# nv-tlabs/GEN3C

Measured on AMD Instinct MI355X. Metric: denoise-steps/sec (121x1280x704 latent, Cosmos-7B), higher is better.
Workload: dtype bf16

## Files before the change

### gen3c_amd/build.py

```python
from __future__ import annotations

import os
import shutil
import subprocess
import sys
from concurrent.futures import ThreadPoolExecutor
from pathlib import Path

ROOT = Path(__file__).resolve().parent
CSRC = ROOT / "csrc"
LIBDIR = ROOT / "lib"
OBJDIR = LIBDIR / "obj"
LIB = LIBDIR / "libgen3c_hip.so"
ARCH = "gfx950"
PER_FILE_FLAGS = {"attention.hip": ("-fno-slp-vectorize",)}


def _hipcc() -> str:
    for cand in (os.environ.get("HIPCC"), shutil.which("hipcc"), "/opt/rocm/bin/hipcc"):
        if cand and Path(cand).exists():
            return cand
    raise RuntimeError("hipcc not found (ROCm toolchain is required to build the gen3c_amd HIP library)")


# ... 5 lines not shown


AUDITED = ("attention", "gemm", "attention_d512")


def _asm_audit(hipcc: str, flags: list, objdir: Path, verbose: bool) -> None:
    root = ROOT.parent
    if not (root / "tools" / "asm_audit.py").exists():
        print("gen3c_amd.build: tools/asm_audit.py not found - inline-asm register audit skipped", file=sys.stderr)
        return
    if str(root) not in sys.path:
        sys.path.insert(0, str(root))
    from tools import asm_audit

    def to_asm(stem: str) -> str:
        out = objdir / (stem + ".audit.s")
        cmd = [hipcc, *flags, *PER_FILE_FLAGS.get(stem + ".hip", ()), "-S", "--cuda-device-only", str(CSRC / (stem + ".hip")), "-o", str(out)]
        if verbose:
            print(" ".join(cmd), flush=True)
        r = subprocess.run(cmd, capture_output=True, text=True)
        if r.returncode != 0:
            raise RuntimeError(f"hipcc -S failed for {stem}.hip:\n{r.stderr}")
        text = out.read_text()
        out.unlink()
        return text

    with ThreadPoolExecutor(max_workers=len(AUDITED)) as ex:
        attn, gemm, d512 = ex.map(to_asm, AUDITED)
    import contextlib
    import io
    buf = io.StringIO()
    with contextlib.redirect_stdout(buf):
        findings = asm_audit.audit(attn) + asm_audit.audit_gemm_w4(gemm) + asm_audit.audit_gemm_w4e(gemm) + asm_audit.audit_attn_d512(d512)
    if verbose:
        print(buf.getvalue())
    if findings:
        raise RuntimeError("inline-asm register audit failed (tools/asm_audit.py):\n" + "\n".join(findings))


def build(verbose: bool = False, force: bool = False, extra_flags: tuple = (), suffix: str = "", audit: bool = True) -> Path:
    hipcc = _hipcc()
    objdir = LIBDIR / ("obj" + suffix)
    lib = LIBDIR / f"libgen3c_hip{suffix}.so"
    objdir.mkdir(parents=True, exist_ok=True)
    headers = sorted(CSRC.glob("*.hpp")) + sorted((ROOT.parent / "include").glob("*.h"))
    sources = sorted(CSRC.glob("*.hip"))
    flags = [f"--offload-arch={ARCH}", "-O3", "-std=c++17", "-fPIC", "-ffp-contract=off", f"-I{ROOT.parent / 'include'}", "-Wall",
             "-Wno-unused-function", *extra_flags]

    stamp = objdir / "asm_audit.ok"
    stale = [src.stem for src in sources if force or _newer(src, objdir / (src.stem + ".o"), headers)]
    audit_future = None
    audit_pool = None
    if audit and not suffix and (not stamp.exists() or any(s_ in AUDITED for s_ in stale)):
        stamp.unlink(missing_ok=True)
        audit_pool = ThreadPoolExecutor(max_workers=1)
        audit_future = audit_pool.submit(_asm_audit, hipcc, flags, objdir, verbose)

    def compile_one(src: Path) -> Path:
        obj = objdir / (src.stem + ".o")
        if src.stem in stale:
            cmd = [hipcc, *flags, *PER_FILE_FLAGS.get(src.name, ()), "-c", str(src), "-o", str(obj)]
            if verbose:
                print(" ".join(cmd), flush=True)
            r = subprocess.run(cmd, capture_output=True, text=True)
            if r.returncode != 0:
# ... 26 lines not shown
```

### gen3c_amd/csrc/attention.hip

```cpp
#include "common.hpp"
#include <stdlib.h>
#include <mutex>
#include <type_traits>

namespace {

constexpr int HD = 128;
constexpr int QB = 32;
constexpr int NWAVES = 8;
constexpr int BQ = QB * NWAVES;
constexpr int KVB = 64;
constexpr int NTHREADS = 64 * NWAVES;

struct AttnParams {
    const bf16_t* Q; int64_t q_row, q_batch, q_head;
    const bf16_t* K; int64_t k_row, k_batch, k_head;
    const bf16_t* Vt; int64_t vt_row, vt_batch, vt_head;
    bf16_t* O; int64_t o_row, o_batch, o_head;
    int Sq, Skv;
    float scale_log2;
    int vt_seg_len;
    int64_t vt_seg_stride;
    int grid_q, n_hb, n_heads, xcd_heads;
    float* O32;
// ... 380 lines not shown
    const float l_tot = xor32_sum(l_run);
    const float inv = 1.0f / l_tot;
    if (q_ok) {
        bf16_t* orow = Ob + (int64_t)q_idx * p.o_row;
#pragma unroll
        for (int d = 0; d < 4; ++d)
#pragma unroll
            for (int q4 = 0; q4 < 4; ++q4) {
                bf16x4 o;
#pragma unroll
                for (int e = 0; e < 4; ++e) o[e] = f32_to_bf16(accO[d][4 * q4 + e] * inv);
                *reinterpret_cast<bf16x4*>(orow + 32 * d + 8 * q4 + 4 * g) = o;
            }
    }
}


template <int OFF> G3_DEVICE void lds_read_frag(bf16x8& dst, uint32_t addr) {
    static_assert(OFF >= 0 && OFF < 65536, "ds_read offset field is 16 bits");
    asm volatile("ds_read_b128 %0, %1 offset:%2" : "=v"(dst) : "v"(addr), "n"(OFF));
}
G3_DEVICE uint32_t lds_addr_flip128(uint32_t a) {
    uint32_t r;
    asm volatile("v_xor_b32 %0, 0x80, %1" : "=v"(r) : "v"(a));
    return r;
}
template <int N> G3_DEVICE void lds_wait_frag(bf16x8& frag) { asm volatile("s_waitcnt lgkmcnt(%1)" : "+v"(frag) : "n"(N)); }

#define G3_SGB(mask, n) __builtin_amdgcn_sched_group_barrier((mask), (n), 0)
constexpr int SGB_VALU = 0x2, SGB_MFMA = 0x8, SGB_DSR = 0x100, SGB_TRANS = 0x400;

#ifndef G3_AB_ATTN_ABLATE
#define G3_AB_ATTN_ABLATE 0
#endif
template <int CTX, int QA, int QBV, bool FOLD, bool MW = false, int MW_RD = 4, int MW_KREGS = 8>
__global__ __launch_bounds__(NTHREADS, 2) void flash_attn_fwd_v3_kernel(AttnParams p) {
    constexpr bool CP = (CTX & 2) != 0;
    extern __shared__ __attribute__((aligned(16))) char smem_raw[];
    bf16_t* sK = reinterpret_cast<bf16_t*>(smem_raw);
    bf16_t* sV = sK + 2 * KVB * HD;

    const int tid = threadIdx.x;
    const int lane = tid & 63;
    const int wave = tid >> 6;
    const int l31 = lane & 31;
    const int g = lane >> 5;
    const int Skv = p.kv_dense > 0 ? p.kv_dense : p.Skv;
    const int head = blockIdx.y;
    const int batch = blockIdx.z;

    const bf16_t* Qb = p.Q + batch * p.q_batch + head * p.q_head;
    const bf16_t* Kb = p.K + batch * p.k_batch + head * p.k_head;
    const bf16_t* Vb = p.Vt + batch * p.vt_batch + head * p.vt_head;
    bf16_t* Ob = p.O + batch * p.o_batch + head * p.o_head;

    const int q_idx = blockIdx.x * BQ + wave * QB + l31;
    const bool q_ok = q_idx < p.Sq;
    bf16x8 qf[8];
    {
        const bf16_t* qrow = Qb + (int64_t)(q_ok ? q_idx : 0) * p.q_row + 8 * g;
#pragma unroll
        for (int ks = 0; ks < 8; ++ks) qf[ks] = q_ok ? load_bf16x8(qrow + 16 * ks) : zero_bf16x8();
        if (p.q_norm_w) {
            float ss = 0.f;
#pragma unroll
            for (int ks = 0; ks < 8; ++ks)
// ... 735 lines not shown
```

### gen3c_amd/csrc/attention_w4.hpp

```cpp

constexpr int W4_WAVES = 4;
constexpr int W4_THREADS = 64 * W4_WAVES;
constexpr int W4_BQ = 64 * W4_WAVES;
constexpr int W4_QBASE = 128;

#define W4_OWNED_AGPRS "a0","a1","a2","a3","a4","a5","a6","a7","a8","a9","a10","a11","a12","a13","a14","a15","a16","a17","a18","a19","a20","a21","a22","a23","a24","a25","a26","a27","a28","a29","a30","a31","a32","a33","a34","a35","a36","a37","a38","a39","a40","a41","a42","a43","a44","a45","a46","a47","a48","a49","a50","a51","a52","a53","a54","a55","a56","a57","a58","a59","a60","a61","a62","a63","a64","a65","a66","a67","a68","a69","a70","a71","a72","a73","a74","a75","a76","a77","a78","a79","a80","a81","a82","a83","a84","a85","a86","a87","a88","a89","a90","a91","a92","a93","a94","a95","a96","a97","a98","a99","a100","a101","a102","a103","a104","a105","a106","a107","a108","a109","a110","a111","a112","a113","a114","a115","a116","a117","a118","a119","a120","a121","a122","a123","a124","a125","a126","a127","a128","a129","a130","a131","a132","a133","a134","a135","a136","a137","a138","a139","a140","a141","a142","a143","a144","a145","a146","a147","a148","a149","a150","a151","a152","a153","a154","a155","a156","a157","a158","a159","a160","a161","a162","a163","a164","a165","a166","a167","a168","a169","a170","a171","a172","a173","a174","a175","a176","a177","a178","a179","a180","a181","a182","a183","a184","a185","a186","a187","a188","a189","a190","a191"

template <int R> G3_DEVICE void w4_acc_zero() { asm volatile("v_accvgpr_write_b32 a%c0, 0" ::"n"(R) : W4_OWNED_AGPRS); }
template <int R> G3_DEVICE void w4_acc_write(uint32_t v) { asm volatile("v_accvgpr_write_b32 a%c1, %0" ::"v"(v), "n"(R) : W4_OWNED_AGPRS); }
template <int R> G3_DEVICE float w4_acc_read() {
    float v;
    asm volatile("v_accvgpr_read_b32 %0, a%c1" : "=v"(v) : "n"(R) : W4_OWNED_AGPRS);
    return v;
}
template <int R> G3_DEVICE void w4_acc_scale(float alpha) {
    float t;
    asm volatile("v_accvgpr_read_b32 %0, a%c2\n\tv_mul_f32 %0, %0, %1\n\tv_accvgpr_write_b32 a%c2, %0" : "=&v"(t) : "v"(alpha), "n"(R) : W4_OWNED_AGPRS);
}
G3_DEVICE void w4_fence_acc() { asm volatile("s_nop 7\n\ts_nop 3" ::: W4_OWNED_AGPRS); }
G3_DEVICE void w4_fence_v(f32x16& a, f32x16& b, f32x16& c, f32x16& d) { asm volatile("s_nop 7\n\ts_nop 3" : "+v"(a), "+v"(b), "+v"(c), "+v"(d)); }

template <int QI, int WAIT> G3_DEVICE void w4_qk(f32x16& S, const bf16x8& kfrag) {
    if constexpr (WAIT >= 0)
        asm volatile("s_waitcnt lgkmcnt(%c4)\n\tv_mfma_f32_32x32x16_bf16 %0, %1, a[%c2:%c3], %0"
                     : "+v"(S) : "v"(kfrag), "n"(W4_QBASE + 4 * QI), "n"(W4_QBASE + 4 * QI + 3), "n"(WAIT) : W4_OWNED_AGPRS);
    else
        asm volatile("v_mfma_f32_32x32x16_bf16 %0, %1, a[%c2:%c3], %0" : "+v"(S) : "v"(kfrag), "n"(W4_QBASE + 4 * QI), "n"(W4_QBASE + 4 * QI + 3) : W4_OWNED_AGPRS);
}
template <int QI, int WAIT> G3_DEVICE void w4_qk0(f32x16& S, const bf16x8& kfrag, const f32x16& c) {
    if constexpr (WAIT >= 0)
        asm volatile("s_waitcnt lgkmcnt(%c5)\n\tv_mfma_f32_32x32x16_bf16 %0, %1, a[%c3:%c4], %2"
                     : "=&v"(S) : "v"(kfrag), "v"(c), "n"(W4_QBASE + 4 * QI), "n"(W4_QBASE + 4 * QI + 3), "n"(WAIT) : W4_OWNED_AGPRS);
    else
        asm volatile("v_mfma_f32_32x32x16_bf16 %0, %1, a[%c3:%c4], %2" : "=&v"(S) : "v"(kfrag), "v"(c), "n"(W4_QBASE + 4 * QI), "n"(W4_QBASE + 4 * QI + 3) : W4_OWNED_AGPRS);
}
template <int OB, int WAIT> G3_DEVICE void w4_pv(const bf16x8& vfrag, const u32x4& pfrag) {
    if constexpr (WAIT >= 0)
        asm volatile("s_waitcnt lgkmcnt(%c4)\n\tv_mfma_f32_32x32x16_bf16 a[%c2:%c3], %0, %1, a[%c2:%c3]" ::"v"(vfrag), "v"(pfrag), "n"(16 * OB), "n"(16 * OB + 15), "n"(WAIT) : W4_OWNED_AGPRS);
    else
        asm volatile("v_mfma_f32_32x32x16_bf16 a[%c2:%c3], %0, %1, a[%c2:%c3]" ::"v"(vfrag), "v"(pfrag), "n"(16 * OB), "n"(16 * OB + 15) : W4_OWNED_AGPRS);
}
G3_DEVICE void w4_dma_piece(uint32_t lds_dst, const char* sbase, uint32_t voff) {
    if (G3_AB_ATTN_ABLATE & 128) return;
    asm volatile("s_mov_b32 m0, %0\n\ts_nop 0\n\tglobal_load_lds_dwordx4 %1, %2" ::"s"(lds_dst), "v"(voff), "s"(sbase) : "memory");
}
template <int OFF> G3_DEVICE void lds_read_frag_flip128(bf16x8& dst, uint32_t addr) {
    uint32_t tmp;
    asm volatile("v_xor_b32 %1, 0x80, %2\n\tds_read_b128 %0, %1 offset:%3" : "=v"(dst), "=&v"(tmp) : "v"(addr), "n"(OFF));
}

#if G3_AB_ATTN_ABLATE & 16
#define W4_UNIT(k) "v_mov_b32 %[k" #k "], 0\n\t"
#else
#define W4_UNIT(k)                                                                                                                      \
    "v_exp_f32 %[a" #k "], %[x" #k "]\n\tv_exp_f32 %[b" #k "], %[y" #k "]\n\tv_add_f32 %[p" #k "], %[p" #k "], %[a" #k "]\n\t"      \
    "v_add_f32 %[r" #k "], %[r" #k "], %[b" #k "]\n\tv_cvt_pk_bf16_f32 %[k" #k "], %[a" #k "], %[b" #k "]\n\t"
#endif
#if G3_AB_ATTN_ABLATE & 32
#define W4_READ ""
#else
#define W4_READ "ds_read_b128 %[nf], %[addr] offset:%c[off]\n\t"
#endif
#ifdef G3_AB_ATTN_EXTRA_NOP
#define W4_WAIT "s_nop 0\n\ts_waitcnt lgkmcnt(%c[wn])\n\t"
#else
#define W4_WAIT "s_waitcnt lgkmcnt(%c[wn])\n\t"
#endif
#define W4_QK(h) "v_mfma_f32_32x32x16_bf16 %[s" #h "], %[f], a[%c[q" #h "]:%c[e" #h "]], %[s" #h "]\n\t"
#define W4_QK0(h) "v_mfma_f32_32x32x16_bf16 %[s" #h "], %[f], a[%c[q" #h "]:%c[e" #h "]], %[c" #h "]\n\t"
#define W4_PV(h) "v_mfma_f32_32x32x16_bf16 a[%c[o" #h "]:%c[g" #h "]], %[f], %[pf" #h "], a[%c[o" #h "]:%c[g" #h "]]\n\t"

struct W4Unit {
    float x, y;
};

template <int QI0, int OFF, int WN, bool INIT, bool TWO>
G3_DEVICE void w4_step_qk(bf16x8& nf, uint32_t addr, const bf16x8& f, f32x16& s0, f32x16& s1, const f32x16& c0, const f32x16& c1, float x1, float y1,
                          uint32_t& k1, float& p1, float& r1, float x2, float y2, uint32_t& k2, float& p2, float& r2) {
    float a1, b1, a2, b2;
    constexpr int q0 = W4_QBASE + 4 * QI0, q1 = W4_QBASE + 4 * (8 + QI0);
#define W4_A_OUT_COMMON [nf] "=&v"(nf), [a1] "=&v"(a1), [b1] "=&v"(b1), [k1] "=&v"(k1), [p1] "+v"(p1), [r1] "+v"(r1)
#define W4_A_OUT_TWO , [a2] "=&v"(a2), [b2] "=&v"(b2), [k2] "=&v"(k2), [p2] "+v"(p2), [r2] "+v"(r2)
#define W4_A_IN_COMMON [f] "v"(f), [addr] "v"(addr), [x1] "v"(x1), [y1] "v"(y1), [off] "n"(OFF), [wn] "n"(WN), [q0] "n"(q0), [e0] "n"(q0 + 3), [q1] "n"(q1), [e1] "n"(q1 + 3)
    if constexpr (INIT && TWO)
        asm volatile(W4_READ W4_WAIT W4_QK0(0) W4_UNIT(1) W4_QK0(1) W4_UNIT(2)
                     : W4_A_OUT_COMMON W4_A_OUT_TWO, [s0] "=&v"(s0), [s1] "=&v"(s1)
                     : W4_A_IN_COMMON, [x2] "v"(x2), [y2] "v"(y2), [c0] "v"(c0), [c1] "v"(c1) : W4_OWNED_AGPRS);
    else if constexpr (INIT && !TWO)
        asm volatile(W4_READ W4_WAIT W4_QK0(0) W4_UNIT(1) W4_QK0(1)
// ... 351 lines not shown
```

### gen3c_amd/csrc/attention_w4b.hpp

```cpp

#ifndef G3_ATTENTION_W4B_HELPERS
#define G3_ATTENTION_W4B_HELPERS
#define W4B_RING_AGPRS "a192","a193","a194","a195","a196","a197","a198","a199","a200","a201","a202","a203","a204","a205","a206","a207","a208","a209","a210","a211","a212","a213","a214","a215","a216","a217","a218","a219","a220","a221","a222","a223","a224","a225","a226","a227","a228","a229","a230","a231","a232","a233","a234","a235","a236","a237","a238","a239","a240","a241","a242","a243","a244","a245","a246","a247","a248","a249","a250","a251","a252","a253","a254","a255"
#define W4B_OWNED W4_OWNED_AGPRS, W4B_RING_AGPRS
constexpr int W4B_RING0 = 192;
constexpr int W4B_D = 6;

#if G3_AB_ATTN_ABLATE & 32
#define W4B_READ ""
#else
#define W4B_READ "ds_read_b128 a[%c[ra]:%c[rb]], %[addr] offset:%c[off]\n\t"
#endif
#define W4B_QK(h) "v_mfma_f32_32x32x16_bf16 %[s" #h "], a[%c[fa]:%c[fb]], a[%c[q" #h "]:%c[e" #h "]], %[s" #h "]\n\t"
#define W4B_QK0(h) "v_mfma_f32_32x32x16_bf16 %[s" #h "], a[%c[fa]:%c[fb]], a[%c[q" #h "]:%c[e" #h "]], %[c" #h "]\n\t"
#define W4B_PV(h) "v_mfma_f32_32x32x16_bf16 a[%c[o" #h "]:%c[g" #h "]], a[%c[fa]:%c[fb]], %[pf" #h "], a[%c[o" #h "]:%c[g" #h "]]\n\t"
#if G3_AB_ATTN_ABLATE & 128
#define W4B_M0 ""
#define W4B_DMA ""
#else
#define W4B_M0 "s_mov_b32 m0, %[m0v]\n\t"
#define W4B_DMA "global_load_lds_dwordx4 %[voff], %[sbase]\n\t"
#endif
#if G3_AB_ATTN_ABLATE & 256
#define W4B_MAXP(k) ""
// ... 21 lines not shown
    constexpr int q0 = W4_QBASE + 4 * ks, q1 = W4_QBASE + 4 * (8 + ks);
    constexpr int fa = W4B_RING0 + 4 * (I & 15), ra = W4B_RING0 + 4 * ((I + W4B_D) & 15);
#define W4B_A_OUT [a1] "+v"(a1), [b1] "+v"(b1), [k1] "=&v"(k1), [p1] "+v"(p1), [r1] "+v"(r1)
#define W4B_A_IN [addr] "v"(addr), [x1] "v"(x1), [y1] "v"(y1), [off] "n"(ROFF), [wn] "n"(WN), [q0] "n"(q0), [e0] "n"(q0 + 3), [q1] "n"(q1), [e1] "n"(q1 + 3), \
                 [fa] "n"(fa), [fb] "n"(fa + 3), [ra] "n"(ra), [rb] "n"(ra + 3)
    static_assert(READ, "region A always reads ahead");
    if constexpr (INIT && DMA)
        asm volatile(W4B_M0 W4B_READ W4_WAIT W4B_QK0(0) W4_UNIT(1) W4B_DMA W4B_QK0(1)
                     : W4B_A_OUT, [s0] "=&v"(s0), [s1] "=&v"(s1) : W4B_A_IN, [c0] "v"(c0), [c1] "v"(c1), [m0v] "s"(m0v), [voff] "v"(voff), [sbase] "s"(sbase)
                     : "memory");
    else if constexpr (!INIT && DMA)
        asm volatile(W4B_M0 W4B_READ W4_WAIT W4B_QK(0) W4_UNIT(1) W4B_DMA W4B_QK(1)
                     : W4B_A_OUT, [s0] "+v"(s0), [s1] "+v"(s1) : W4B_A_IN, [m0v] "s"(m0v), [voff] "v"(voff), [sbase] "s"(sbase) : "memory");
    else if constexpr (INIT && !DMA && EXTRA == 1)
        asm volatile(W4B_READ W4_WAIT W4B_QK0(0) W4_UNIT(1) W4B_QK0(1) W4B_XA
                     : W4B_A_OUT, [s0] "=&v"(s0), [s1] "=&v"(s1), [a2] "=&v"(*a2), [b2] "=&v"(*b2), [pe] "+v"(*pe)
                     : W4B_A_IN, [c0] "v"(c0), [c1] "v"(c1), [x2] "v"(x2), [y2] "v"(y2));
    else if constexpr (INIT && !DMA)
        asm volatile(W4B_READ W4_WAIT W4B_QK0(0) W4_UNIT(1) W4B_QK0(1)
                     : W4B_A_OUT, [s0] "=&v"(s0), [s1] "=&v"(s1) : W4B_A_IN, [c0] "v"(c0), [c1] "v"(c1));
    else if constexpr (EXTRA == 1)
        asm volatile(W4B_READ W4_WAIT W4B_QK(0) W4_UNIT(1) W4B_QK(1) W4B_XA
                     : W4B_A_OUT, [s0] "+v"(s0), [s1] "+v"(s1), [a2] "=&v"(*a2), [b2] "=&v"(*b2), [pe] "+v"(*pe) : W4B_A_IN, [x2] "v"(x2), [y2] "v"(y2));
    else if constexpr (EXTRA == 2)
        asm volatile(W4B_READ W4_WAIT W4B_QK(0) W4_UNIT(1) W4B_QK(1) W4B_XB
                     : W4B_A_OUT, [s0] "+v"(s0), [s1] "+v"(s1), [k2] "=&v"(*k2), [pe] "+v"(*pe) : W4B_A_IN, [a2] "v"(*a2), [b2] "v"(*b2));
    else
        asm volatile(W4B_READ W4_WAIT W4B_QK(0) W4_UNIT(1) W4B_QK(1) : W4B_A_OUT, [s0] "+v"(s0), [s1] "+v"(s1) : W4B_A_IN);
    static_assert(EXTRA == 0 || (!DMA && !(INIT && EXTRA == 2)), "w4b_step_qk: extra half units only on steps without an LDS-DMA piece");
#undef W4B_A_OUT
#undef W4B_A_IN
}

template <int I, int ROFF, bool READ, int WN, bool UNIT, int MX>
G3_DEVICE void w4b_step_pv(uint32_t addr, const u32x4& pf0, const u32x4& pf1, float x1, float y1, uint32_t& k1, float& p1, float& r1, float& mx, float& my,
                           float ma0, float mb0, float mc0, float md0, float ma1, float mb1, float mc1, float md1, float ma2, float mb2, float mc2, float md2,
                           float& a1, float& b1) {
    constexpr int D = I & 3;
    constexpr int o0 = 16 * D, o1 = 16 * (4 + D);
    constexpr int fa = W4B_RING0 + 4 * ((16 + I) & 15), ra = W4B_RING0 + 4 * ((16 + I + W4B_D) & 15);
#define W4B_B_IN [pf0] "v"(pf0), [pf1] "v"(pf1), [wn] "n"(WN), [o0] "n"(o0), [g0] "n"(o0 + 15), [o1] "n"(o1), [g1] "n"(o1 + 15), [fa] "n"(fa), [fb] "n"(fa + 3)
#define W4B_B_RD [addr] "v"(addr), [off] "n"(ROFF), [ra] "n"(ra), [rb] "n"(ra + 3)
#define W4B_B_UO [a1] "+v"(a1), [b1] "+v"(b1), [k1] "=&v"(k1), [p1] "+v"(p1), [r1] "+v"(r1)
#define W4B_B_UI [x1] "v"(x1), [y1] "v"(y1)
#define W4B_B_M0 [ma0] "v"(ma0), [mb0] "v"(mb0), [mc0] "v"(mc0), [md0] "v"(md0)
    if constexpr (READ && UNIT && MX == 0)
        asm volatile(W4B_READ W4_WAIT W4B_PV(0) W4_UNIT(1) W4B_PV(1) : W4B_B_UO : W4B_B_IN, W4B_B_RD, W4B_B_UI);
    else if constexpr (READ && UNIT && MX == 1)
        asm volatile(W4B_READ W4_WAIT W4B_PV(0) W4_UNIT(1) W4B_PV(1) W4B_MAXP0(0) : W4B_B_UO, [mx] "=&v"(mx), [my] "=&v"(my) : W4B_B_IN, W4B_B_RD, W4B_B_UI, W4B_B_M0);
    else if constexpr (READ && UNIT && MX == 2)
        asm volatile(W4B_READ W4_WAIT W4B_PV(0) W4_UNIT(1) W4B_PV(1) W4B_MAXP(0) : W4B_B_UO, [mx] "+v"(mx), [my] "+v"(my) : W4B_B_IN, W4B_B_RD, W4B_B_UI, W4B_B_M0);
    else if constexpr (!READ && UNIT && MX == 1)
        asm volatile(W4_WAIT W4B_PV(0) W4_UNIT(1) W4B_PV(1) W4B_MAXP0(0) : W4B_B_UO, [mx] "=&v"(mx), [my] "=&v"(my) : W4B_B_IN, W4B_B_UI, W4B_B_M0);
    else if constexpr (!READ && UNIT && MX == 2)
        asm volatile(W4_WAIT W4B_PV(0) W4_UNIT(1) W4B_PV(1) W4B_MAXP(0) : W4B_B_UO, [mx] "+v"(mx), [my] "+v"(my) : W4B_B_IN, W4B_B_UI, W4B_B_M0);
    else if constexpr (!READ && UNIT && MX == 0)
        asm volatile(W4_WAIT W4B_PV(0) W4_UNIT(1) W4B_PV(1) : W4B_B_UO : W4B_B_IN, W4B_B_UI);
    else if constexpr (!READ && !UNIT && MX == 3)
        asm volatile(W4_WAIT W4B_PV(0) W4B_MAXP(0) W4B_PV(1) W4B_MAXP(1) W4B_MAXP(2)
                     : [mx] "+v"(mx), [my] "+v"(my)
                     : W4B_B_IN, W4B_B_M0, [ma1] "v"(ma1), [mb1] "v"(mb1), [mc1] "v"(mc1), [md1] "v"(md1), [ma2] "v"(ma2), [mb2] "v"(mb2), [mc2] "v"(mc2), [md2] "v"(md2));
    else if constexpr (READ && !UNIT && MX == 3)
        asm volatile(W4B_READ W4_WAIT W4B_PV(0) W4B_MAXP(0) W4B_PV(1) W4B_MAXP(1) W4B_MAXP(2)
                     : [mx] "+v"(mx), [my] "+v"(my)
                     : W4B_B_IN, W4B_B_RD, W4B_B_M0, [ma1] "v"(ma1), [mb1] "v"(mb1), [mc1] "v"(mc1), [md1] "v"(md1), [ma2] "v"(ma2), [mb2] "v"(mb2), [mc2] "v"(mc2), [md2] "v"(md2));
    else if constexpr (READ && !UNIT && MX == 0)
        asm volatile(W4B_READ W4_WAIT W4B_PV(0) W4B_PV(1) : : W4B_B_IN, W4B_B_RD);
    else {
        static_assert(!READ && !UNIT && MX == 0, "w4b_step_pv: combination not laid out");
        asm volatile(W4_WAIT W4B_PV(0) W4B_PV(1) : : W4B_B_IN);
    }
#undef W4B_B_RD
#undef W4B_B_UO
#undef W4B_B_UI
#undef W4B_B_M0
}
template <int I, int WN, bool READ = false, int ROFF = 0>
G3_DEVICE void w4b_step_pv_fold(const u32x4& pf0, const u32x4& pf1, float& a0, float& b0, float& c0, float& d0, float& a1, float& b1, float& c1, float& d1, float& t0,
                                 float& t1, uint32_t addr = 0u) {
    constexpr int D = I & 3;
    constexpr int o0 = 16 * D, o1 = 16 * (4 + D);
    constexpr int fa = W4B_RING0 + 4 * ((16 + I) & 15), ra = W4B_RING0 + 4 * ((16 + I + W4B_D) & 15);
    if constexpr (READ && I == 14)
        asm volatile(W4B_READ W4_WAIT W4B_PV(0) "v_max3_f32 %[a0], %[a0], %[b0], %[c0]\n\tv_max3_f32 %[a1], %[a1], %[b1], %[c1]\n\tv_max_f32 %[a0], %[a0], %[d0]\n\tv_max_f32 %[a1], %[a1], %[d1]\n\t"
                     W4B_PV(1) "v_mov_b32 %[t0], %[a0]\n\tv_mov_b32 %[t1], %[a1]\n\t"
                     : [a0] "+v"(a0), [a1] "+v"(a1), [t0] "=&v"(t0), [t1] "=&v"(t1)
                     : W4B_B_IN, [b0] "v"(b0), [c0] "v"(c0), [d0] "v"(d0), [b1] "v"(b1), [c1] "v"(c1), [d1] "v"(d1), [addr] "v"(addr), [off] "n"(ROFF), [ra] "n"(ra), [rb] "n"(ra + 3));
    else if constexpr (READ)
        asm volatile(W4B_READ W4_WAIT W4B_PV(0) "v_permlane32_swap_b32 %[t0], %[a0]\n\tv_permlane32_swap_b32 %[t1], %[a1]\n\t" W4B_PV(1)
                     "v_max_f32 %[a0], %[a0], %[t0]\n\tv_max_f32 %[a1], %[a1], %[t1]\n\t"
                     : [a0] "+v"(a0), [a1] "+v"(a1), [t0] "+v"(t0), [t1] "+v"(t1) : W4B_B_IN, [addr] "v"(addr), [off] "n"(ROFF), [ra] "n"(ra), [rb] "n"(ra + 3));
    else if constexpr (I == 14)
        asm volatile(W4_WAIT W4B_PV(0) "v_max3_f32 %[a0], %[a0], %[b0], %[c0]\n\tv_max3_f32 %[a1], %[a1], %[b1], %[c1]\n\tv_max_f32 %[a0], %[a0], %[d0]\n\tv_max_f32 %[a1], %[a1], %[d1]\n\t"
                     W4B_PV(1) "v_mov_b32 %[t0], %[a0]\n\tv_mov_b32 %[t1], %[a1]\n\t"
                     : [a0] "+v"(a0), [a1] "+v"(a1), [t0] "=&v"(t0), [t1] "=&v"(t1)
                     : W4B_B_IN, [b0] "v"(b0), [c0] "v"(c0), [d0] "v"(d0), [b1] "v"(b1), [c1] "v"(c1), [d1] "v"(d1));
    else
        asm volatile(W4_WAIT W4B_PV(0) "v_permlane32_swap_b32 %[t0], %[a0]\n\tv_permlane32_swap_b32 %[t1], %[a1]\n\t" W4B_PV(1)
                     "v_max_f32 %[a0], %[a0], %[t0]\n\tv_max_f32 %[a1], %[a1], %[t1]\n\t"
                     : [a0] "+v"(a0), [a1] "+v"(a1), [t0] "+v"(t0), [t1] "+v"(t1) : W4B_B_IN);
}
#undef W4B_B_IN

G3_DEVICE void w4b_fence_acc() { asm volatile("s_nop 7\n\ts_nop 3" ::: W4B_OWNED); }
template <int R> G3_DEVICE void w4b_sub_inplace(f32x16& x, float d) {
    float t = x[R];
    asm volatile("v_sub_f32 %0, %0, %1" : "+v"(t) : "v"(d));
    x[R] = t;
}
template <int R> G3_DEVICE void w4b_set_inplace(f32x16& x, float v) {
    float t = x[R];
    asm volatile("v_mov_b32 %0, %1" : "+v"(t) : "v"(v));
    x[R] = t;
}
G3_DEVICE void w4b_mul_inplace(float& x, float a) { asm volatile("v_mul_f32 %0, %0, %1" : "+v"(x) : "v"(a)); }

#endif

#if W4B_CP
#define W4B_KERNEL flash_attn_fwd_w4b_carry_kernel
#else
#define W4B_KERNEL flash_attn_fwd_w4b_kernel
#endif
template <bool XB>
__global__ __launch_bounds__(W4_THREADS, 1) void W4B_KERNEL(AttnParams p) {
    constexpr bool CP = W4B_CP;
    extern __shared__ __attribute__((aligned(16))) char smem_raw[];
    bf16_t* sK = reinterpret_cast<bf16_t*>(smem_raw);
    bf16_t* sV = sK + 2 * KVB * HD;

    const int tid = threadIdx.x;
    const int lane = tid & 63;
    const int wave = __builtin_amdgcn_readfirstlane(tid >> 6);
    const int l31 = lane & 31;
    const int g = lane >> 5;
    int qblk = blockIdx.x, head = blockIdx.y, batch = blockIdx.z;
    if (p.xcd_heads) {
        const int xcd = blockIdx.x & 7, slot = blockIdx.x >> 3;
        const int hb = xcd + 8 * (slot / p.grid_q);
        qblk = slot - (slot / p.grid_q) * p.grid_q;
        head = hb % p.n_heads;
        batch = hb / p.n_heads;
    }

    const bf16_t* Qb = p.Q + batch * p.q_batch + head * p.q_head;
    const bf16_t* Kb = p.K + batch * p.k_batch + head * p.k_head;
    const bf16_t* Vb = p.Vt + batch * p.vt_batch + head * p.vt_head;
    bf16_t* Ob = p.O + batch * p.o_batch + head * p.o_head;
    float* o32_base = p.O32;
    float* lse_base = p.LSE;
    asm volatile("" : "+s"(o32_base), "+s"(lse_base));
    const float* carry_o = nullptr;
    const float* carry_lse = nullptr;
    uint32_t skip_t0 = 0u, skip_nt = 0u, v_skip = 0u;
    if constexpr (CP) {
        carry_o = p.carry_o;
        carry_lse = p.carry_lse;
        skip_t0 = (uint32_t)p.kv_skip_begin / KVB;
        skip_nt = (uint32_t)p.kv_skip_len / KVB;
// ... 173 lines not shown
        }
        u32x4 pb[2][4];
        auto ux = [&](auto uc) -> float { constexpr int u = decltype(uc)::value, sl = u >> 3, h = (u >> 2) & 1, q = u & 3; return S_cur[h][sl >> 1][(sl & 1) * 8 + 2 * q]; };
        auto uy = [&](auto uc) -> float { constexpr int u = decltype(uc)::value, sl = u >> 3, h = (u >> 2) & 1, q = u & 3; return S_cur[h][sl >> 1][(sl & 1) * 8 + 2 * q + 1]; };
        auto uput = [&](auto uc, uint32_t pk) { constexpr int u = decltype(uc)::value, sl = u >> 3, h = (u >> 2) & 1, q = u & 3; pb[h][sl][q] = pk; };
        auto sm_unit = [&](auto uc) {
            constexpr int u = decltype(uc)::value, h = (u >> 2) & 1, pa = 2 * (u & 1);
            float a, b;
            uint32_t pk;
            if (G3_AB_ATTN_ABLATE & 16) {
                pk = 0;
            } else {
                asm volatile("v_exp_f32 %0, %5\n\tv_exp_f32 %1, %6\n\tv_add_f32 %3, %3, %0\n\tv_add_f32 %4, %4, %1\n\tv_cvt_pk_bf16_f32 %2, %0, %1"
                             : "=&v"(a), "=&v"(b), "=v"(pk), "+v"(psum[h][pa]), "+v"(psum[h][pa + 1]) : "v"(ux(uc)), "v"(uy(uc)));
            }
            uput(uc, pk);
        };
        constexpr int NHEAD = has_next ? (XB ? 0 : 4) : 20;
        static_for<0, NHEAD>([&](auto uc) { sm_unit(uc); });

        if constexpr (has_next) {
            const int t2 = min(t + 2, nt - 1);
            const char* kbase = Kbytes + k_tile((uint32_t)t2) * k_tile_bytes;
            const char* vbase = Vbytes + v_off_next;
            static_for<0, 16>([&](auto ic) {
                constexpr int I = decltype(ic)::value;
                using NR = std::integral_constant<int, I + D>;
                using U = std::integral_constant<int, (XB ? 0 : 4) + I>;
                constexpr int hu = (U::value >> 2) & 1, pa = 2 * (I & 1);
                constexpr bool dma = XB ? (I & 1) == 0 : I < 8;
                constexpr int j = XB ? (I >> 1) : (I & 7);
                const uint32_t m0v = dma ? (j < 4 ? lds_k0 + (uint32_t)(par * KVB * HD * 2 + 256 * j * 16) : lds_v0 + (uint32_t)((par ^ 1) * HD * KVB * 2 + 256 * (j - 4) * 16)) + (uint32_t)wave * 1024u : 0u;
                uint32_t k1 = 0;
                if constexpr (XB && (I & 1)) {
                    constexpr int ex = (I & 2) ? 2 : 1;
                    constexpr int xu = 16 + (I >> 2);
                    using XU = std::integral_constant<int, xu>;
                    uint32_t k2 = 0;
                    w4b_step_qk<I, frag_off(NR{}), true, D, (I >> 1) == 0, false, ex>(frag_addr(NR{}), S_next[0][I & 1], S_next[1][I & 1], negm[0], negm[1], ux(U{}), uy(U{}), k1,
                                                                                      psum[hu][pa], psum[hu][pa + 1], 0u, 0u, nullptr, ta[I & 1], tb[I & 1], ux(XU{}), uy(XU{}), &k2,
                                                                                      &pe[0][ex - 1], &xa[0], &xb[0]);
                    if constexpr (ex == 2) uput(XU{}, k2);
                } else {
                    w4b_step_qk<I, frag_off(NR{}), true, D, (I >> 1) == 0, dma>(frag_addr(NR{}), S_next[0][I & 1], S_next[1][I & 1], negm[0], negm[1], ux(U{}), uy(U{}), k1,
                                                                               psum[hu][pa], psum[hu][pa + 1], m0v, dma_off[j], j < 4 ? kbase : vbase, ta[I & 1], tb[I & 1]);
                }
                uput(U{}, k1);
            });
            const bool wrap = (v_seg_pos + 1u == seg_tiles);
            v_off_next += wrap ? (uint32_t)(KVB * 2) + v_seg_jump : (uint32_t)(KVB * 2);
            v_seg_pos = wrap ? 0u : v_seg_pos + 1u;
            if constexpr (CP) v_off_next += (uint32_t)(t + 2) == skip_t0 ? v_skip : 0u;
        }
        G3_JITTER(wave + blockIdx.x + 3, t);
        {
            float cx[2][2], cy[2][2], tx[2];
            auto sn = [&](auto hc, auto mbc, auto rc) -> float { return S_next[decltype(hc)::value][decltype(mbc)::value][decltype(rc)::value]; };
            constexpr int KSN = par * KVB * HD * 2;
            auto rd_off = [](auto nc) constexpr { constexpr int n = decltype(nc)::value; return n < 32 ? VS + 32 * ((n - 16) & 3) * KVB * 2 : KSN + 32 * (n & 1) * HD * 2; };
            auto rd_addr = [&](auto nc) -> uint32_t { constexpr int n = decltype(nc)::value; if constexpr (n < 32) return vaddr[((n - 16) >> 2) & 3]; else return kaddr[((n - 32) >> 1) & 7]; };
            static_for<0, 14>([&](auto ic) {
                constexpr int I = decltype(ic)::value;
                constexpr bool rd = (I + D < 16) || (XB && has_next);
                using NR = std::integral_constant<int, rd ? 16 + I + D : 16>;
                constexpr bool unit = I < 12;
                using U = std::integral_constant<int, unit ? 20 + I : 20>;
                constexpr int hu = (U::value >> 2) & 1, pa = 2 * (I & 1);
                constexpr int mxk = !has_next ? 0 : (I < 2 ? 0 : (I == 2 || I == 3 || I == 10 || I == 11) ? 1 : I < 12 ? 2 : 3);
                constexpr int mh = I < 10 ? 0 : 1;
                constexpr int k0 = I < 2 ? 0 : I < 10 ? I - 2 : I < 12 ? I - 10 : I == 12 ? 2 : 5;
                constexpr int k1i = mxk == 3 ? k0 + 1 : k0, k2i = mxk == 3 ? k0 + 2 : k0;
                using H = std::integral_constant<int, mh>;
#define W4B_SN(mb, r) (has_next ? sn(H{}, std::integral_constant<int, mb>{}, std::integral_constant<int, (r)>{}) : 0.f)
                if constexpr (XB && has_next && I == 10) {
                    if (!(G3_AB_ATTN_ABLATE & 64)) asm volatile("s_waitcnt vmcnt(0)\n\ts_barrier" ::: "memory");
                }
                uint32_t k1 = 0;
                w4b_step_pv<I, rd_off(NR{}), rd, rd ? D : 15 - I, unit, mxk>(rd_addr(NR{}), pb[0][I >> 2], pb[1][I >> 2], ux(U{}), uy(U{}), k1, psum[hu][pa], psum[hu][pa + 1],
                                                                          cx[mh][I & 1], cy[mh][I & 1], W4B_SN(0, 2 * k0), W4B_SN(0, 2 * k0 + 1), W4B_SN(1, 2 * k0),
                                                                          W4B_SN(1, 2 * k0 + 1), W4B_SN(0, 2 * k1i), W4B_SN(0, 2 * k1i + 1), W4B_SN(1, 2 * k1i),
                                                                          W4B_SN(1, 2 * k1i + 1), W4B_SN(0, 2 * k2i), W4B_SN(0, 2 * k2i + 1), W4B_SN(1, 2 * k2i),
                                                                          W4B_SN(1, 2 * k2i + 1), ta[I & 1], tb[I & 1]);
#undef W4B_SN
                if constexpr (unit) uput(U{}, k1);
            });
            if constexpr (has_next) {
                if constexpr (XB) {
                    using N14 = std::integral_constant<int, 16 + 14 + D>;
                    using N15 = std::integral_constant<int, 16 + 15 + D>;
                    w4b_step_pv_fold<14, D, true, rd_off(N14{})>(pb[0][3], pb[1][3], cx[0][0], cy[0][0], cx[0][1], cy[0][1], cx[1][0], cy[1][0], cx[1][1], cy[1][1], tx[0], tx[1],
                                                                 rd_addr(N14{}));
                    w4b_step_pv_fold<15, D, true, rd_off(N15{})>(pb[0][3], pb[1][3], cx[0][0], cy[0][0], cx[0][1], cy[0][1], cx[1][0], cy[1][0], cx[1][1], cy[1][1], tx[0], tx[1],
                                                                 rd_addr(N15{}));
                } else {
                    w4b_step_pv_fold<14, 1>(pb[0][3], pb[1][3], cx[0][0], cy[0][0], cx[0][1], cy[0][1], cx[1][0], cy[1][0], cx[1][1], cy[1][1], tx[0], tx[1]);
                    w4b_step_pv_fold<15, 0>(pb[0][3], pb[1][3], cx[0][0], cy[0][0], cx[0][1], cy[0][1], cx[1][0], cy[1][0], cx[1][1], cy[1][1], tx[0], tx[1]);
                }
                mx_cur[0] = cx[0][0];
                mx_cur[1] = cx[1][0];
            } else {
                float d0 = 0.f, d1 = 0.f;
                uint32_t kd = 0;
                w4b_step_pv<14, 0, false, 1, false, 0>(0u, pb[0][3], pb[1][3], 0.f, 0.f, kd, d0, d1, d0, d1, 0, 0, 0, 0, 0, 0, 0, 0, 0, 0, 0, 0, d0, d1);
                w4b_step_pv<15, 0, false, 0, false, 0>(0u, pb[0][3], pb[1][3], 0.f, 0.f, kd, d0, d1, d0, d1, 0, 0, 0, 0, 0, 0, 0, 0, 0, 0, 0, 0, d0, d1);
            }
        }
        if (!XB && has_next && !(G3_AB_ATTN_ABLATE & 64)) lds_dma_publish_barrier();
    };

    using True = std::integral_constant<bool, true>;
    using False = std::integral_constant<bool, false>;
    using P0 = std::integral_constant<int, 0>;
    using P1 = std::integral_constant<int, 1>;
    int t = 0;
    for (; t + 2 < nt; t += 2) {
        tile(SA, SB, t, True{}, P0{});
        tile(SB, SA, t + 1, True{}, P1{});
    }
    if (t + 1 < nt) {
        tile(SA, SB, t, True{}, P0{});
        tile(SB, SA, t + 1, False{}, P1{});
    } else {
        tile(SA, SB, t, False{}, P0{});
    }

// ... 82 lines not shown
```

Measured before the change: 0.2968.

## Space LDS waits and interleave exp units between MFMAs in w4b attention

Adds spaced variants of the w4b QK and PV step functions that split each exp/softmax unit into an exp half and an accumulate/pack half placed around the two MFMAs. Every other step skips its LDS wait, and the extra exp work is distributed across steps. The aim is to hide transcendental and LDS latency behind matrix ops in the XB non-CP kernel path. It is on by default behind a G3_AB_ATTN_SPACING macro, and a new build-time assembly audit checks the spacing. Relaxing the waits risks reading fragments before they have landed if the ordering assumptions are wrong.

```diff
diff --git a/gen3c_amd/build.py b/gen3c_amd/build.py
--- a/gen3c_amd/build.py
+++ b/gen3c_amd/build.py
@@ -61,6 +61,7 @@
     buf = io.StringIO()
     with contextlib.redirect_stdout(buf):
         findings = asm_audit.audit(attn) + asm_audit.audit_gemm_w4(gemm) + asm_audit.audit_gemm_w4e(gemm) + asm_audit.audit_attn_d512(d512)
+        findings += asm_audit.audit_w4b_spacing(attn, check=asm_audit.W4B_SPACING_ENFORCED and "-DG3_AB_ATTN_SPACING=0" not in flags)
     if verbose:
         print(buf.getvalue())
     if findings:
diff --git a/gen3c_amd/csrc/attention.hip b/gen3c_amd/csrc/attention.hip
--- a/gen3c_amd/csrc/attention.hip
+++ b/gen3c_amd/csrc/attention.hip
@@ -436,6 +436,9 @@
 
 #ifndef G3_AB_ATTN_ABLATE
 #define G3_AB_ATTN_ABLATE 0
+#endif
+#ifndef G3_AB_ATTN_SPACING
+#define G3_AB_ATTN_SPACING 1
 #endif
 template <int CTX, int QA, int QBV, bool FOLD, bool MW = false, int MW_RD = 4, int MW_KREGS = 8>
 __global__ __launch_bounds__(NTHREADS, 2) void flash_attn_fwd_v3_kernel(AttnParams p) {
diff --git a/gen3c_amd/csrc/attention_w4.hpp b/gen3c_amd/csrc/attention_w4.hpp
--- a/gen3c_amd/csrc/attention_w4.hpp
+++ b/gen3c_amd/csrc/attention_w4.hpp
@@ -55,6 +55,14 @@
 #define W4_UNIT(k)                                                                                                                      \
     "v_exp_f32 %[a" #k "], %[x" #k "]\n\tv_exp_f32 %[b" #k "], %[y" #k "]\n\tv_add_f32 %[p" #k "], %[p" #k "], %[a" #k "]\n\t"      \
     "v_add_f32 %[r" #k "], %[r" #k "], %[b" #k "]\n\tv_cvt_pk_bf16_f32 %[k" #k "], %[a" #k "], %[b" #k "]\n\t"
+#endif
+#if G3_AB_ATTN_ABLATE & 16
+#define W4_UNIT_E(k) ""
+#define W4_UNIT_P(k) "v_mov_b32 %[k" #k "], 0\n\t"
+#else
+#define W4_UNIT_E(k) "v_exp_f32 %[a" #k "], %[x" #k "]\n\tv_exp_f32 %[b" #k "], %[y" #k "]\n\t"
+#define W4_UNIT_P(k) \
+    "v_add_f32 %[p" #k "], %[p" #k "], %[a" #k "]\n\tv_add_f32 %[r" #k "], %[r" #k "], %[b" #k "]\n\tv_cvt_pk_bf16_f32 %[k" #k "], %[a" #k "], %[b" #k "]\n\t"
 #endif
 #if G3_AB_ATTN_ABLATE & 32
 #define W4_READ ""
diff --git a/gen3c_amd/csrc/attention_w4b.hpp b/gen3c_amd/csrc/attention_w4b.hpp
--- a/gen3c_amd/csrc/attention_w4b.hpp
+++ b/gen3c_amd/csrc/attention_w4b.hpp
@@ -77,6 +77,49 @@
 #undef W4B_A_IN
 }
 
+#define W4B_X1 "v_exp_f32 %[a2], %[x2]\n\t"
+#define W4B_X2 "v_add_f32 %[pe], %[pe], %[a2]\n\t"
+#define W4B_X3 "v_exp_f32 %[b2], %[x2]\n\t"
+#define W4B_X4 "v_add_f32 %[pe], %[pe], %[b2]\n\t"
+#define W4B_X4K "v_cvt_pk_bf16_f32 %[k2], %[a2], %[b2]\n\t"
+#define W4B_SP_ASM(head, tail, ...)                                  \
+    do {                                                             \
+        if constexpr (WN >= 0) asm volatile(head W4_WAIT tail __VA_ARGS__); \
+        else asm volatile(head tail __VA_ARGS__);                    \
+    } while (0)
+template <int I, int ROFF, int WN, bool INIT, bool DMA, int XM>
+G3_DEVICE void w4b_step_qk_sp(uint32_t addr, f32x16& s0, f32x16& s1, const f32x16& c0, const f32x16& c1, float x1, float y1, uint32_t& k1, float& p1, float& r1,
+                              uint32_t m0v, uint32_t voff, const char* sbase, float& a1, float& b1, float x2, uint32_t& k2, float& pe, float& a2, float& b2) {
+    constexpr int ks = I >> 1;
+    constexpr int q0 = W4_QBASE + 4 * ks, q1 = W4_QBASE + 4 * (8 + ks);
+    constexpr int fa = W4B_RING0 + 4 * (I & 15), ra = W4B_RING0 + 4 * ((I + W4B_D) & 15);
+#define W4B_A_OUT [a1] "+v"(a1), [b1] "+v"(b1), [k1] "=&v"(k1), [p1] "+v"(p1), [r1] "+v"(r1)
+#define W4B_A_IN [addr] "v"(addr), [x1] "v"(x1), [y1] "v"(y1), [off] "n"(ROFF), [wn] "n"(WN < 0 ? 0 : WN), [q0] "n"(q0), [e0] "n"(q0 + 3), [q1] "n"(q1), [e1] "n"(q1 + 3), \
+                 [fa] "n"(fa), [fb] "n"(fa + 3), [ra] "n"(ra), [rb] "n"(ra + 3)
+#define W4B_A_DMA [m0v] "s"(m0v), [voff] "v"(voff), [sbase] "s"(sbase)
+    if constexpr (INIT && DMA && XM == 0)
+        W4B_SP_ASM(W4B_M0 W4B_READ, W4B_QK0(0) W4_UNIT_E(1) W4B_DMA W4B_QK0(1) W4_UNIT_P(1),
+                   : W4B_A_OUT, [s0] "=&v"(s0), [s1] "=&v"(s1) : W4B_A_IN, [c0] "v"(c0), [c1] "v"(c1), W4B_A_DMA : "memory");
+    else if constexpr (INIT && !DMA && XM == 1)
+        W4B_SP_ASM(W4B_READ, W4B_QK0(0) W4_UNIT_E(1) W4B_X1 W4B_QK0(1) W4_UNIT_P(1),
+                   : W4B_A_OUT, [s0] "=&v"(s0), [s1] "=&v"(s1), [a2] "=&v"(a2) : W4B_A_IN, [c0] "v"(c0), [c1] "v"(c1), [x2] "v"(x2));
+    else if constexpr (!INIT && !DMA && XM == 1)
+        W4B_SP_ASM(W4B_READ, W4B_QK(0) W4_UNIT_E(1) W4B_X1 W4B_QK(1) W4_UNIT_P(1), : W4B_A_OUT, [s0] "+v"(s0), [s1] "+v"(s1), [a2] "=&v"(a2) : W4B_A_IN, [x2] "v"(x2));
+    else if constexpr (!INIT && DMA && XM == 2)
+        W4B_SP_ASM(W4B_M0 W4B_READ, W4B_QK(0) W4_UNIT_E(1) W4B_X2 W4B_DMA W4B_QK(1) W4_UNIT_P(1),
+                   : W4B_A_OUT, [s0] "+v"(s0), [s1] "+v"(s1), [pe] "+v"(pe) : W4B_A_IN, W4B_A_DMA, [a2] "v"(a2) : "memory");
+    else if constexpr (!INIT && !DMA && XM == 3)
+        W4B_SP_ASM(W4B_READ, W4B_QK(0) W4_UNIT_E(1) W4B_X3 W4B_QK(1) W4_UNIT_P(1), : W4B_A_OUT, [s0] "+v"(s0), [s1] "+v"(s1), [b2] "=&v"(b2) : W4B_A_IN, [x2] "v"(x2));
+    else {
+        static_assert(!INIT && DMA && XM == 4, "w4b_step_qk_sp: combination not laid out");
+        W4B_SP_ASM(W4B_M0 W4B_READ, W4B_QK(0) W4_UNIT_E(1) W4B_X4 W4B_DMA W4B_QK(1) W4_UNIT_P(1) W4B_X4K,
+                   : W4B_A_OUT, [s0] "+v"(s0), [s1] "+v"(s1), [pe] "+v"(pe), [k2] "=&v"(k2) : W4B_A_IN, W4B_A_DMA, [a2] "v"(a2), [b2] "v"(b2) : "memory");
+    }
+#undef W4B_A_OUT
+#undef W4B_A_IN
+#undef W4B_A_DMA
+}
+
 template <int I, int ROFF, bool READ, int WN, bool UNIT, int MX>
 G3_DEVICE void w4b_step_pv(uint32_t addr, const u32x4& pf0, const u32x4& pf1, float x1, float y1, uint32_t& k1, float& p1, float& r1, float& mx, float& my,
                            float ma0, float mb0, float mc0, float md0, float ma1, float mb1, float mc1, float md1, float ma2, float mb2, float mc2, float md2,
@@ -84,7 +127,7 @@
     constexpr int D = I & 3;
     constexpr int o0 = 16 * D, o1 = 16 * (4 + D);
     constexpr int fa = W4B_RING0 + 4 * ((16 + I) & 15), ra = W4B_RING0 + 4 * ((16 + I + W4B_D) & 15);
-#define W4B_B_IN [pf0] "v"(pf0), [pf1] "v"(pf1), [wn] "n"(WN), [o0] "n"(o0), [g0] "n"(o0 + 15), [o1] "n"(o1), [g1] "n"(o1 + 15), [fa] "n"(fa), [fb] "n"(fa + 3)
+#define W4B_B_IN [pf0] "v"(pf0), [pf1] "v"(pf1), [wn] "n"(WN < 0 ? 0 : WN), [o0] "n"(o0), [g0] "n"(o0 + 15), [o1] "n"(o1), [g1] "n"(o1 + 15), [fa] "n"(fa), [fb] "n"(fa + 3)
 #define W4B_B_RD [addr] "v"(addr), [off] "n"(ROFF), [ra] "n"(ra), [rb] "n"(ra + 3)
 #define W4B_B_UO [a1] "+v"(a1), [b1] "+v"(b1), [k1] "=&v"(k1), [p1] "+v"(p1), [r1] "+v"(r1)
 #define W4B_B_UI [x1] "v"(x1), [y1] "v"(y1)
@@ -115,18 +158,45 @@
         static_assert(!READ && !UNIT && MX == 0, "w4b_step_pv: combination not laid out");
         asm volatile(W4_WAIT W4B_PV(0) W4B_PV(1) : : W4B_B_IN);
     }
+}
+template <int I, int ROFF, int WN, bool UNIT, int MX, bool XT>
+G3_DEVICE void w4b_step_pv_sp(uint32_t addr, const u32x4& pf0, const u32x4& pf1, float x1, float y1, uint32_t& k1, float& p1, float& r1, float& mx, float& my,
+                              float ma0, float mb0, float mc0, float md0, float ma1, float mb1, float mc1, float md1, float ma2, float mb2, float mc2, float md2,
+                              float& a1, float& b1, uint32_t& k2, float& pe, float a2, float b2) {
+    constexpr int D = I & 3;
+    constexpr int o0 = 16 * D, o1 = 16 * (4 + D);
+    constexpr int fa = W4B_RING0 + 4 * ((16 + I) & 15), ra = W4B_RING0 + 4 * ((16 + I + W4B_D) & 15);
+    if constexpr (UNIT && MX == 0 && XT)
+        W4B_SP_ASM(W4B_READ, W4B_PV(0) W4_UNIT_E(1) W4B_X4 W4B_PV(1) W4_UNIT_P(1) W4B_X4K,
+                   : W4B_B_UO, [pe] "+v"(pe), [k2] "=&v"(k2) : W4B_B_IN, W4B_B_RD, W4B_B_UI, [a2] "v"(a2), [b2] "v"(b2));
+    else if constexpr (UNIT && MX == 0)
+        W4B_SP_ASM(W4B_READ, W4B_PV(0) W4_UNIT_E(1) W4B_PV(1) W4_UNIT_P(1), : W4B_B_UO : W4B_B_IN, W4B_B_RD, W4B_B_UI);
+    else if constexpr (UNIT && MX == 1)
+        W4B_SP_ASM(W4B_READ, W4B_PV(0) W4_UNIT_E(1) W4B_MAXP0(0) W4B_PV(1) W4_UNIT_P(1), : W4B_B_UO, [mx] "=&v"(mx), [my] "=&v"(my) : W4B_B_IN, W4B_B_RD, W4B_B_UI, W4B_B_M0);
+    else if constexpr (UNIT && MX == 2)
+        W4B_SP_ASM(W4B_READ, W4B_PV(0) W4_UNIT_E(1) W4B_MAXP(0) W4B_PV(1) W4_UNIT_P(1), : W4B_B_UO, [mx] "+v"(mx), [my] "+v"(my) : W4B_B_IN, W4B_B_RD, W4B_B_UI, W4B_B_M0);
+    else {
+        static_assert(!UNIT && MX == 3 && !XT, "w4b_step_pv_sp: combination not laid out");
+        W4B_SP_ASM(W4B_READ, W4B_PV(0) W4B_MAXP(0) W4B_MAXP(1) W4B_PV(1) W4B_MAXP(2),
+                   : [mx] "+v"(mx), [my] "+v"(my)
+                   : W4B_B_IN, W4B_B_RD, W4B_B_M0, [ma1] "v"(ma1), [mb1] "v"(mb1), [mc1] "v"(mc1), [md1] "v"(md1), [ma2] "v"(ma2), [mb2] "v"(mb2), [mc2] "v"(mc2), [md2] "v"(md2));
+    }
+}
 #undef W4B_B_RD
 #undef W4B_B_UO
 #undef W4B_B_UI
 #undef W4B_B_M0
-}
 template <int I, int WN, bool READ = false, int ROFF = 0>
 G3_DEVICE void w4b_step_pv_fold(const u32x4& pf0, const u32x4& pf1, float& a0, float& b0, float& c0, float& d0, float& a1, float& b1, float& c1, float& d1, float& t0,
                                  float& t1, uint32_t addr = 0u) {
     constexpr int D = I & 3;
     constexpr int o0 = 16 * D, o1 = 16 * (4 + D);
     constexpr int fa = W4B_RING0 + 4 * ((16 + I) & 15), ra = W4B_RING0 + 4 * ((16 + I + W4B_D) & 15);
-    if constexpr (READ && I == 14)
+    if constexpr (READ && I == 15 && WN < 0)
+        asm volatile(W4B_READ W4B_PV(0) "v_permlane32_swap_b32 %[t0], %[a0]\n\tv_permlane32_swap_b32 %[t1], %[a1]\n\t" W4B_PV(1)
+                     "v_max_f32 %[a0], %[a0], %[t0]\n\tv_max_f32 %[a1], %[a1], %[t1]\n\t"
+                     : [a0] "+v"(a0), [a1] "+v"(a1), [t0] "+v"(t0), [t1] "+v"(t1) : W4B_B_IN, [addr] "v"(addr), [off] "n"(ROFF), [ra] "n"(ra), [rb] "n"(ra + 3));
+    else if constexpr (READ && I == 14)
         asm volatile(W4B_READ W4_WAIT W4B_PV(0) "v_max3_f32 %[a0], %[a0], %[b0], %[c0]\n\tv_max3_f32 %[a1], %[a1], %[b1], %[c1]\n\tv_max_f32 %[a0], %[a0], %[d0]\n\tv_max_f32 %[a1], %[a1], %[d1]\n\t"
                      W4B_PV(1) "v_mov_b32 %[t0], %[a0]\n\tv_mov_b32 %[t1], %[a1]\n\t"
                      : [a0] "+v"(a0), [a1] "+v"(a1), [t0] "=&v"(t0), [t1] "=&v"(t1)
@@ -170,6 +240,7 @@
 template <bool XB>
 __global__ __launch_bounds__(W4_THREADS, 1) void W4B_KERNEL(AttnParams p) {
     constexpr bool CP = W4B_CP;
+    constexpr bool SPACED = XB && !W4B_CP && G3_AB_ATTN_SPACING;
     extern __shared__ __attribute__((aligned(16))) char smem_raw[];
     bf16_t* sK = reinterpret_cast<bf16_t*>(smem_raw);
     bf16_t* sV = sK + 2 * KVB * HD;
@@ -409,7 +480,15 @@
                 constexpr int j = XB ? (I >> 1) : (I & 7);
                 const uint32_t m0v = dma ? (j < 4 ? lds_k0 + (uint32_t)(par * KVB * HD * 2 + 256 * j * 16) : lds_v0 + (uint32_t)((par ^ 1) * HD * KVB * 2 + 256 * (j - 4) * 16)) + (uint32_t)wave * 1024u : 0u;
                 uint32_t k1 = 0;
-                if constexpr (XB && (I & 1)) {
+                if constexpr (SPACED) {
+                    constexpr int xm = I == 0 ? 0 : (I & 3) == 0 ? 4 : (I & 3);
+                    using XU = std::integral_constant<int, I == 0 ? 16 : 16 + ((I - 1) >> 2)>;
+                    uint32_t k2 = 0;
+                    w4b_step_qk_sp<I, frag_off(NR{}), ((I & 1) ? -1 : D - 1), (I >> 1) == 0, dma, xm>(frag_addr(NR{}), S_next[0][I & 1], S_next[1][I & 1], negm[0], negm[1], ux(U{}), uy(U{}), k1,
+                                                                                 psum[hu][pa], psum[hu][pa + 1], m0v, dma_off[j], j < 4 ? kbase : vbase, ta[I & 1], tb[I & 1],
+                                                                                 xm == 3 ? uy(XU{}) : ux(XU{}), k2, pe[0][xm == 2 ? 0 : 1], xa[0], xb[0]);
+                    if constexpr (xm == 4) uput(XU{}, k2);
+                } else if constexpr (XB && (I & 1)) {
                     constexpr int ex = (I & 2) ? 2 : 1;
                     constexpr int xu = 16 + (I >> 2);
                     using XU = std::integral_constant<int, xu>;
@@ -453,11 +532,21 @@
                     if (!(G3_AB_ATTN_ABLATE & 64)) asm volatile("s_waitcnt vmcnt(0)\n\ts_barrier" ::: "memory");
                 }
                 uint32_t k1 = 0;
-                w4b_step_pv<I, rd_off(NR{}), rd, rd ? D : 15 - I, unit, mxk>(rd_addr(NR{}), pb[0][I >> 2], pb[1][I >> 2], ux(U{}), uy(U{}), k1, psum[hu][pa], psum[hu][pa + 1],
+                if constexpr (SPACED && has_next) {
+                    uint32_t k2 = 0;
+                    w4b_step_pv_sp<I, rd_off(NR{}), ((I & 1) ? -1 : D - 1), unit, mxk, I == 0>(rd_addr(NR{}), pb[0][I >> 2], pb[1][I >> 2], ux(U{}), uy(U{}), k1, psum[hu][pa], psum[hu][pa + 1],
+                                                                          cx[mh][I & 1], cy[mh][I & 1], W4B_SN(0, 2 * k0), W4B_SN(0, 2 * k0 + 1), W4B_SN(1, 2 * k0),
+                                                                          W4B_SN(1, 2 * k0 + 1), W4B_SN(0, 2 * k1i), W4B_SN(0, 2 * k1i + 1), W4B_SN(1, 2 * k1i),
+                                                                          W4B_SN(1, 2 * k1i + 1), W4B_SN(0, 2 * k2i), W4B_SN(0, 2 * k2i + 1), W4B_SN(1, 2 * k2i),
+                                                                          W4B_SN(1, 2 * k2i + 1), ta[I & 1], tb[I & 1], k2, pe[0][1], xa[0], xb[0]);
+                    if constexpr (I == 0) uput(std::integral_constant<int, 19>{}, k2);
+                } else {
+                    w4b_step_pv<I, rd_off(NR{}), rd, rd ? D : 15 - I, unit, mxk>(rd_addr(NR{}), pb[0][I >> 2], pb[1][I >> 2], ux(U{}), uy(U{}), k1, psum[hu][pa], psum[hu][pa + 1],
                                                                           cx[mh][I & 1], cy[mh][I & 1], W4B_SN(0, 2 * k0), W4B_SN(0, 2 * k0 + 1), W4B_SN(1, 2 * k0),
                                                                           W4B_SN(1, 2 * k0 + 1), W4B_SN(0, 2 * k1i), W4B_SN(0, 2 * k1i + 1), W4B_SN(1, 2 * k1i),
                                                                           W4B_SN(1, 2 * k1i + 1), W4B_SN(0, 2 * k2i), W4B_SN(0, 2 * k2i + 1), W4B_SN(1, 2 * k2i),
                                                                           W4B_SN(1, 2 * k2i + 1), ta[I & 1], tb[I & 1]);
+                }
 #undef W4B_SN
                 if constexpr (unit) uput(U{}, k1);
             });
@@ -465,9 +554,9 @@
                 if constexpr (XB) {
                     using N14 = std::integral_constant<int, 16 + 14 + D>;
                     using N15 = std::integral_constant<int, 16 + 15 + D>;
-                    w4b_step_pv_fold<14, D, true, rd_off(N14{})>(pb[0][3], pb[1][3], cx[0][0], cy[0][0], cx[0][1], cy[0][1], cx[1][0], cy[1][0], cx[1][1], cy[1][1], tx[0], tx[1],
+                    w4b_step_pv_fold<14, (SPACED ? D - 1 : D), true, rd_off(N14{})>(pb[0][3], pb[1][3], cx[0][0], cy[0][0], cx[0][1], cy[0][1], cx[1][0], cy[1][0], cx[1][1], cy[1][1], tx[0], tx[1],
                                                                  rd_addr(N14{}));
-                    w4b_step_pv_fold<15, D, true, rd_off(N15{})>(pb[0][3], pb[1][3], cx[0][0], cy[0][0], cx[0][1], cy[0][1], cx[1][0], cy[1][0], cx[1][1], cy[1][1], tx[0], tx[1],
+                    w4b_step_pv_fold<15, (SPACED ? -1 : D), true, rd_off(N15{})>(pb[0][3], pb[1][3], cx[0][0], cy[0][0], cx[0][1], cy[0][1], cx[1][0], cy[1][0], cx[1][1], cy[1][1], tx[0], tx[1],
                                                                  rd_addr(N15{}));
                 } else {
                     w4b_step_pv_fold<14, 1>(pb[0][3], pb[1][3], cx[0][0], cy[0][0], cx[0][1], cy[0][1], cx[1][0], cy[1][0], cx[1][1], cy[1][1], tx[0], tx[1]);
```

After: 0.2997 (median of 6 runs). No clear change (+1.0%).
